# PolarisRisingWar/rgb-experiment

Hardware: AMD Instinct MI355X
Metric: aggregated edges/sec (full-graph GCN d=128, reference epoch = train fwd+bwd+Adam + 2 eval fwd) (higher is better)
Workload: dtype f32

## Files before the change

rgb_experiment_amd/csrc/gemm.hip:

```cpp
#include "rgbx_common.h"

namespace rgbx {
namespace {

constexpr int BM = 128, BN = 128, KT = 32;
enum { A_PLAIN = 0, A_BN = 1, A_ROWS = 2 };

struct TnExtra {
  const float* X;
  int64_t ldx;
  const float *mean, *rstd, *ca, *cb, *ck;
  const int32_t* rows;
  int64_t n_rows;
};
using f32x16 = __attribute__((ext_vector_type(16))) float;

template <int W>
__device__ __forceinline__ void stage_tile(float* __restrict__ lds, const float* __restrict__ src,
                                           int64_t ld, int64_t k0, int64_t k_end, int c0, int ncols) {
  const int tid = threadIdx.x;
#pragma unroll 4
  for (int p = 0; p < KT * W / 256; ++p) {
    const int idx = p * 256 + tid;
    const int r = idx / W, c = idx % W;
    const int64_t k = k0 + r;
    lds[r * W + c] = (k < k_end && c0 + c < ncols) ? src[k * ld + c0 + c] : 0.f;
  }
}

template <int W>
__device__ __forceinline__ void fetch_tile(float4 (&regs)[KT * (W / 4) / 256], const float* __restrict__ src, int64_t ld,
                                           int64_t k0, int64_t k_end, int c0, int ncols) {
#pragma unroll
  for (int p = 0; p < KT * (W / 4) / 256; ++p) {
    const int idx = p * 256 + threadIdx.x;
    const int r = idx / (W / 4), c = (idx % (W / 4)) * 4;
    const int64_t k = k0 + r;
    regs[p] = make_float4(0.f, 0.f, 0.f, 0.f);
    if (k < k_end && c0 + c < ncols) regs[p] = *reinterpret_cast<const float4*>(src + k * ld + c0 + c);
  }
}

template <int W>
__device__ __forceinline__ void put_tile(float* __restrict__ lds, const float4 (&regs)[KT * (W / 4) / 256]) {
#pragma unroll
  for (int p = 0; p < KT * (W / 4) / 256; ++p) {
    const int idx = p * 256 + threadIdx.x;
    const int r = idx / (W / 4), c = (idx % (W / 4)) * 4;
    *reinterpret_cast<float4*>(lds + r * W + c) = regs[p];
  }
}

template <int W>
__device__ __forceinline__ void put_tile_bn(float* __restrict__ lds, const float4 (&rg)[KT * (W / 4) / 256],
                                            const float4 (&rx)[KT * (W / 4) / 256], const float* __restrict__ lc,
                                            int64_t k0, int64_t k_end, int c0, int ncols) {
#pragma unroll
  for (int p = 0; p < KT * (W / 4) / 256; ++p) {
    const int idx = p * 256 + threadIdx.x;
    const int r = idx / (W / 4), c = (idx % (W / 4)) * 4;
    float4 v = rg[p];
    if (k0 + r < k_end && c0 + c < ncols) {
      const float4 mu = *reinterpret_cast<const float4*>(lc + 0 * W + c);
      const float4 rs = *reinterpret_cast<const float4*>(lc + 1 * W + c);
      const float4 a = *reinterpret_cast<const float4*>(lc + 2 * W + c);
      const float4 b = *reinterpret_cast<const float4*>(lc + 3 * W + c);
      const float4 k = *reinterpret_cast<const float4*>(lc + 4 * W + c);
      v.x = bn_bwd_input_grad(v.x, rx[p].x, mu.x, rs.x, a.x, b.x, k.x);
      v.y = bn_bwd_input_grad(v.y, rx[p].y, mu.y, rs.y, a.y, b.y, k.y);
      v.z = bn_bwd_input_grad(v.z, rx[p].z, mu.z, rs.z, a.z, b.z, k.z);
      v.w = bn_bwd_input_grad(v.w, rx[p].w, mu.w, rs.w, a.w, b.w, k.w);
    }
    *reinterpret_cast<float4*>(lds + r * W + c) = v;
  }
}

template <int W>
__device__ __forceinline__ void fetch_row_ids(int32_t (&ids)[KT * (W / 4) / 256], const int32_t* __restrict__ rows,
                                              int64_t j0, int64_t j_end) {
#pragma unroll
  for (int p = 0; p < KT * (W / 4) / 256; ++p) {
    const int64_t j = j0 + (p * 256 + (int)threadIdx.x) / (W / 4);
    ids[p] = j < j_end ? rows[j] : -1;
  }
}

template <int W>
__device__ __forceinline__ void fetch_tile_rows(float4 (&regs)[KT * (W / 4) / 256], const float* __restrict__ src,
                                                int64_t ld, const int32_t (&ids)[KT * (W / 4) / 256], int c0, int ncols) {
#pragma unroll
  for (int p = 0; p < KT * (W / 4) / 256; ++p) {
    const int c = ((p * 256 + (int)threadIdx.x) % (W / 4)) * 4;
    regs[p] = make_float4(0.f, 0.f, 0.f, 0.f);
    if (ids[p] >= 0 && c0 + c < ncols) regs[p] = *reinterpret_cast<const float4*>(src + (int64_t)ids[p] * ld + c0 + c);
  }
}

__device__ __forceinline__ int64_t lower_bound_rows(const int32_t* __restrict__ rows, int64_t n, int64_t key) {
  int64_t lo = 0, hi = n;
  while (lo < hi) {
    const int64_t mid = (lo + hi) >> 1;
    if (rows[mid] < key) lo = mid + 1; else hi = mid;
  }
  return lo;
}

template <bool VEC4, int MT, int MODE = A_PLAIN>
__global__ void __launch_bounds__(256)
gemm_tn_partial_kernel(const float* __restrict__ A, int64_t lda, const float* __restrict__ B, int64_t ldb,
                       float* __restrict__ part, float* __restrict__ colpart, int64_t K, int M, int N,
                       int64_t slab, TnExtra ex) {
  static_assert(MODE == A_PLAIN || VEC4, "the A_BN / A_ROWS forms exist on the 16-byte path only");
  constexpr int MI = MT / 64;
  __shared__ float lds[KT * (MT + 128) + (MODE == A_BN ? 5 * MT : 0)];
  float* la = lds;
  float* lb = lds + KT * MT;
  const int split = blockIdx.x;
  const int m0 = blockIdx.y * MT, n0 = blockIdx.z * BN;
  const int64_t k_begin = (int64_t)split * slab;
  const int64_t k_end = k_begin + slab < K ? k_begin + slab : K;
  const int wave = threadIdx.x >> 6, lane = threadIdx.x & 63;
  const int wm = (wave >> 1) * (MT / 2), wn = (wave & 1) * 64;
  const int kr = lane >> 5, cc = lane & 31;

  f32x16 acc[MI][2];
#pragma unroll
  for (int i = 0; i < MI; ++i)
#pragma unroll
    for (int j = 0; j < 2; ++j)
#pragma unroll
      for (int r = 0; r < 16; ++r) acc[i][j][r] = 0.f;

  const bool sums = colpart != nullptr && blockIdx.z == 0 && threadIdx.x < MT;
  float csum = 0.f;
  auto consume = [&]() {
    if (sums) {
#pragma unroll 8
      for (int r = 0; r < KT; ++r) csum += la[r * MT + threadIdx.x];
    }
#pragma unroll 4
    for (int kk = 0; kk < KT; kk += 2) {
      float a[MI];
#pragma unroll
      for (int i = 0; i < MI; ++i) a[i] = la[(kk + kr) * MT + wm + i * 32 + cc];
      const float b0 = lb[(kk + kr) * 128 + wn + cc];
      const float b1 = lb[(kk + kr) * 128 + wn + 32 + cc];
#pragma unroll
      for (int i = 0; i < MI; ++i) {
        acc[i][0] = __builtin_amdgcn_mfma_f32_32x32x2f32(a[i], b0, acc[i][0], 0, 0, 0);
        acc[i][1] = __builtin_amdgcn_mfma_f32_32x32x2f32(a[i], b1, acc[i][1], 0, 0, 0);
      }
    }
  };
  if constexpr (MODE == A_BN) {
    float* lc = lds + KT * (MT + 128);
    for (int i = threadIdx.x; i < 5 * MT; i += 256) {
      const float* src = i < MT ? ex.mean : i < 2 * MT ? ex.rstd : i < 3 * MT ? ex.ca : i < 4 * MT ? ex.cb : ex.ck;
      const int c = m0 + i % MT;
      lc[i] = c < M ? src[c] : 0.f;
    }
    float4 ra[KT * (MT / 4) / 256], rx[KT * (MT / 4) / 256], rb[KT * 32 / 256];
    fetch_tile<MT>(ra, A, lda, k_begin, k_end, m0, M);
    fetch_tile<MT>(rx, ex.X, ex.ldx, k_begin, k_end, m0, M);
    fetch_tile<128>(rb, B, ldb, k_begin, k_end, n0, N);
    for (int64_t k0 = k_begin; k0 < k_end; k0 += KT) {
      __syncthreads();
      put_tile_bn<MT>(la, ra, rx, lc, k0, k_end, m0, M);
      put_tile<128>(lb, rb);
      __syncthreads();
      if (k0 + KT < k_end) {
        fetch_tile<MT>(ra, A, lda, k0 + KT, k_end, m0, M);
        fetch_tile<MT>(rx, ex.X, ex.ldx, k0 + KT, k_end, m0, M);
        fetch_tile<128>(rb, B, ldb, k0 + KT, k_end, n0, N);
      }
      consume();
    }
  } else if constexpr (MODE == A_ROWS) {
    const int64_t j_begin = lower_bound_rows(ex.rows, ex.n_rows, k_begin);
    const int64_t j_end = lower_bound_rows(ex.rows, ex.n_rows, k_end);
    float4 ra[KT * (MT / 4) / 256], rb[KT * 32 / 256];
    int32_t ia[KT * (MT / 4) / 256], ib[KT * 32 / 256];
    fetch_row_ids<MT>(ia, ex.rows, j_begin, j_end);
    fetch_row_ids<128>(ib, ex.rows, j_begin, j_end);
    fetch_tile_rows<MT>(ra, A, lda, ia, m0, M);
    fetch_tile_rows<128>(rb, B, ldb, ib, n0, N);
    fetch_row_ids<MT>(ia, ex.rows, j_begin + KT, j_end);
    fetch_row_ids<128>(ib, ex.rows, j_begin + KT, j_end);
    for (int64_t j0 = j_begin; j0 < j_end; j0 += KT) {
      __syncthreads();
      put_tile<MT>(la, ra);
      put_tile<128>(lb, rb);
      __syncthreads();
      if (j0 + KT < j_end) {
        fetch_tile_rows<MT>(ra, A, lda, ia, m0, M);
        fetch_tile_rows<128>(rb, B, ldb, ib, n0, N);
        fetch_row_ids<MT>(ia, ex.rows, j0 + 2 * KT, j_end);
        fetch_row_ids<128>(ib, ex.rows, j0 + 2 * KT, j_end);
      }
      consume();
    }
  } else if constexpr (VEC4) {
    float4 ra[KT * (MT / 4) / 256], rb[KT * 32 / 256];
    fetch_tile<MT>(ra, A, lda, k_begin, k_end, m0, M);
    fetch_tile<128>(rb, B, ldb, k_begin, k_end, n0, N);
    for (int64_t k0 = k_begin; k0 < k_end; k0 += KT) {
      __syncthreads();
      put_tile<MT>(la, ra);
      put_tile<128>(lb, rb);
      __syncthreads();
      if (k0 + KT < k_end) {
        fetch_tile<MT>(ra, A, lda, k0 + KT, k_end, m0, M);
        fetch_tile<128>(rb, B, ldb, k0 + KT, k_end, n0, N);
      }
      consume();
    }
  } else {
    for (int64_t k0 = k_begin; k0 < k_end; k0 += KT) {
      __syncthreads();
      stage_tile<MT>(la, A, lda, k0, k_end, m0, M);
      stage_tile<128>(lb, B, ldb, k0, k_end, n0, N);
      __syncthreads();
      consume();
    }
  }

  if (sums && m0 + (int)threadIdx.x < M) colpart[(int64_t)split * M + m0 + threadIdx.x] = csum;
  float* out = part + (int64_t)split * M * N;
#pragma unroll
  for (int i = 0; i < MI; ++i)
#pragma unroll
    for (int j = 0; j < 2; ++j)
#pragma unroll
      for (int r = 0; r < 16; ++r) {
        const int m = m0 + wm + i * 32 + (r & 3) + 8 * (r >> 2) + 4 * kr;
        const int n = n0 + wn + j * 32 + cc;
        if (m < M && n < N) out[(int64_t)m * N + n] = acc[i][j][r];
      }
}

__global__ void __launch_bounds__(256)
gemm_tn_reduce_kernel(const float* __restrict__ part, int S, int64_t MN, float* __restrict__ C, int N,
                      int64_t ldc, float alpha) {
  __shared__ float sh[8][32];
  const int j = threadIdx.x & 31, q = threadIdx.x >> 5;
  for (int64_t base = (int64_t)blockIdx.x * 32; base < MN; base += (int64_t)gridDim.x * 32) {
    const int64_t i = base + j;
    float s = 0.f;
    if (i < MN)
      for (int p = q; p < S; p += 8) s += part[(int64_t)p * MN + i];
    __syncthreads();
    sh[q][j] = s;
    __syncthreads();
    if (q == 0 && i < MN) {
      float t = 0.f;
#pragma unroll
      for (int k = 0; k < 8; ++k) t += sh[k][j];
      C[(i / N) * ldc + (i % N)] = alpha * t;
    }
  }
}

int tile_rows(int M) { return M <= 64 ? 64 : BM; }

int choose_splits(int64_t K, int M, int N) {
  const int64_t tiles = cdiv(M, tile_rows(M)) * cdiv(N, BN);
  int64_t s = cdiv(tile_rows(M) == 64 ? 1024 : 768, tiles);
  const int64_t max_s = cdiv(K, 16 * KT);
  if (s > max_s) s = max_s;
  if (s < 1) s = 1;
  return (int)s;
}

}
}

using namespace rgbx;

extern "C" int rgbx_gemm_tn_workspace_bytes(int64_t K, int64_t M, int64_t N, size_t* bytes) {
  if (!bytes || K < 0 || M < 0 || N < 0) return fail(RGBX_E_ARG, "gemm_tn_workspace_bytes: bad argument");
  if (M >= INT32_MAX || N >= INT32_MAX) return fail(RGBX_E_RANGE, "gemm_tn: M or N exceeds int32");
  *bytes = (size_t)choose_splits(K, (int)M, (int)N) * ((size_t)M * (size_t)N + (size_t)M) * sizeof(float);
  return RGBX_OK;
}

namespace rgbx {
namespace {

int run_gemm_tn(const char* name, int mode, const float* A, int64_t lda, const float* B, int64_t ldb, float* C,
                int64_t ldc, float* a_colsum, int64_t K, int64_t M, int64_t N, float alpha, void* workspace,
                size_t workspace_bytes, rgbx_stream_t stream, const TnExtra& ex) {
  if (K < 0 || M < 0 || N < 0) return fail(RGBX_E_ARG, "%s: negative size", name);
  if (M == 0 || N == 0) return RGBX_OK;
  if (!C || (K > 0 && (!A || !B))) return fail(RGBX_E_ARG, "%s: null pointer", name);
  if (M >= INT32_MAX || N >= INT32_MAX) return fail(RGBX_E_RANGE, "%s: M or N exceeds int32", name);
  if (lda < M || ldb < N || ldc < N) return fail(RGBX_E_ARG, "%s: leading dimension too small", name);
  bool v4 = aligned16(A) && aligned16(B) && lda % 4 == 0 && ldb % 4 == 0;
  if (mode == A_BN) {
    if (K > 0 && (!ex.X || !ex.mean || !ex.rstd || !ex.ca || !ex.cb || !ex.ck))
      return fail(RGBX_E_ARG, "%s: null pointer", name);
    if (ex.ldx < M) return fail(RGBX_E_ARG, "%s: leading dimension too small", name);
    v4 = v4 && aligned16(ex.X) && ex.ldx % 4 == 0;
  }
  if (mode == A_ROWS) {
    if (ex.n_rows < 0 || ex.n_rows > K || (ex.n_rows > 0 && !ex.rows)) return fail(RGBX_E_ARG, "%s: bad row list", name);
    if (K >= INT32_MAX) return fail(RGBX_E_RANGE, "%s: K exceeds int32", name);
  }
  if (mode != A_PLAIN && !v4)
    return fail(RGBX_E_ALIGN, "%s: operands must be 16-byte aligned with leading dimensions that are multiples of 4", name);
  size_t need = 0;
  if (int rc = rgbx_gemm_tn_workspace_bytes(K, M, N, &need)) return rc;
  if (!workspace || workspace_bytes < need)
    return fail(RGBX_E_WS, "%s: workspace %zu < %zu bytes", name, workspace_bytes, need);
  hipStream_t s = (hipStream_t)stream;
  const int S = choose_splits(K, (int)M, (int)N);
  const int64_t slab = cdiv(cdiv(K > 0 ? K : 1, S), KT) * KT;
  float* part = static_cast<float*>(workspace);
  float* colpart = a_colsum ? part + (size_t)S * M * N : nullptr;
  const int mt = tile_rows((int)M);
  dim3 grid(S, (unsigned)cdiv(M, mt), (unsigned)cdiv(N, BN));
#define RGBX_GEMM_TN(V4, MT, MODE) \
  gemm_tn_partial_kernel<V4, MT, MODE><<<grid, 256, 0, s>>>(A, lda, B, ldb, part, colpart, K, (int)M, (int)N, slab, ex)
  if (mode == A_BN) { if (mt == 64) RGBX_GEMM_TN(true, 64, A_BN); else RGBX_GEMM_TN(true, 128, A_BN); }
  else if (mode == A_ROWS) { if (mt == 64) RGBX_GEMM_TN(true, 64, A_ROWS); else RGBX_GEMM_TN(true, 128, A_ROWS); }
  else if (v4) { if (mt == 64) RGBX_GEMM_TN(true, 64, A_PLAIN); else RGBX_GEMM_TN(true, 128, A_PLAIN); }
  else { if (mt == 64) RGBX_GEMM_TN(false, 64, A_PLAIN); else RGBX_GEMM_TN(false, 128, A_PLAIN); }
#undef RGBX_GEMM_TN
  RGBX_CHECK_LAUNCH("gemm_tn_partial_kernel");
  const int64_t MN = M * N;
  int64_t rb = cdiv(MN, 32);
  if (rb > kMaxGrid) rb = kMaxGrid;
  gemm_tn_reduce_kernel<<<(int)rb, 256, 0, s>>>(part, S, MN, C, (int)N, ldc, alpha);
  RGBX_CHECK_LAUNCH("gemm_tn_reduce_kernel");
  if (a_colsum) {
    gemm_tn_reduce_kernel<<<(int)cdiv(M, 32), 256, 0, s>>>(colpart, S, M, a_colsum, (int)M, M, 1.0f);
    RGBX_CHECK_LAUNCH("gemm_tn_reduce_kernel");
  }
  return RGBX_OK;
}

}
}

extern "C" int rgbx_gemm_tn_f32(const float* A, int64_t lda, const float* B, int64_t ldb, float* C,
                                int64_t ldc, float* a_colsum, int64_t K, int64_t M, int64_t N, float alpha,
                                void* workspace, size_t workspace_bytes, rgbx_stream_t stream) {
  return run_gemm_tn("gemm_tn", A_PLAIN, A, lda, B, ldb, C, ldc, a_colsum, K, M, N, alpha, workspace, workspace_bytes,
                     stream, TnExtra{});
}

extern "C" int rgbx_gemm_tn_bn_bwd_f32(const float* G, int64_t ldg, const float* X, int64_t ldx, const float* mean,
                                       const float* rstd, const float* ca, const float* cb, const float* ck,
                                       const float* B, int64_t ldb, float* C, int64_t ldc, float* a_colsum, int64_t K,
                                       int64_t M, int64_t N, float alpha, void* workspace, size_t workspace_bytes,
                                       rgbx_stream_t stream) {
  TnExtra ex{};
  ex.X = X, ex.ldx = ldx, ex.mean = mean, ex.rstd = rstd, ex.ca = ca, ex.cb = cb, ex.ck = ck;
  return run_gemm_tn("gemm_tn_bn_bwd", A_BN, G, ldg, B, ldb, C, ldc, a_colsum, K, M, N, alpha, workspace,
                     workspace_bytes, stream, ex);
}

extern "C" int rgbx_gemm_tn_rows_f32(const float* A, int64_t lda, const float* B, int64_t ldb, const int32_t* rows,
                                     int64_t n_rows, float* C, int64_t ldc, float* a_colsum, int64_t K, int64_t M,
                                     int64_t N, float alpha, void* workspace, size_t workspace_bytes,
                                     rgbx_stream_t stream) {
  TnExtra ex{};
  ex.rows = rows, ex.n_rows = n_rows;
  return run_gemm_tn("gemm_tn_rows", A_ROWS, A, lda, B, ldb, C, ldc, a_colsum, K, M, N, alpha, workspace,
                     workspace_bytes, stream, ex);
}
```

Before: 17.06 billion.

## Software-pipeline MFMA LDS reads, set waves_per_eu, and merge split-K reductions

Adds a rotated consume loop for the 128-row tile that prefetches the next k-step's A/B operands from LDS between MFMA issues, pinned in place with sched_barrier, so LDS latency overlaps matrix work. Sets an amdgpu_waves_per_eu hint (3 for the BN 128-tile variant, 1 otherwise) to steer register allocation. The split-K reduce kernel now handles both the C reduction and the column-sum reduction in a single launch, and unrolls its partial-sum loads 8-way to raise memory-level parallelism. The gains depend on the compiler honouring the scheduling barriers, and the waves_per_eu hint may change occupancy.

```diff
diff --git a/rgb_experiment_amd/csrc/gemm.hip b/rgb_experiment_amd/csrc/gemm.hip
--- a/rgb_experiment_amd/csrc/gemm.hip
+++ b/rgb_experiment_amd/csrc/gemm.hip
@@ -106,7 +106,7 @@
 }
 
 template <bool VEC4, int MT, int MODE = A_PLAIN>
-__global__ void __launch_bounds__(256)
+__global__ void __launch_bounds__(256) __attribute__((amdgpu_waves_per_eu(MODE == A_BN && MT == 128 ? 3 : 1)))
 gemm_tn_partial_kernel(const float* __restrict__ A, int64_t lda, const float* __restrict__ B, int64_t ldb,
                        float* __restrict__ part, float* __restrict__ colpart, int64_t K, int M, int N,
                        int64_t slab, TnExtra ex) {
@@ -152,6 +152,36 @@
       }
     }
   };
+  auto consume_rotate = [&]() {
+    constexpr int I1 = MI - 1;
+    if (sums) {
+#pragma unroll 8
+      for (int r = 0; r < KT; ++r) csum += la[r * MT + threadIdx.x];
+    }
+    const float* pa = la + kr * MT + wm + cc;
+    const float* pb = lb + kr * 128 + wn + cc;
+    float a0 = pa[0], a1 = pa[I1 * 32], b0 = pb[0], b1 = pb[32];
+#pragma unroll
+    for (int kk = 2; kk <= KT; kk += 2) {
+      const bool more = kk < KT;
+      __builtin_amdgcn_sched_barrier(0);
+      acc[0][0] = __builtin_amdgcn_mfma_f32_32x32x2f32(a0, b0, acc[0][0], 0, 0, 0);
+      acc[0][1] = __builtin_amdgcn_mfma_f32_32x32x2f32(a0, b1, acc[0][1], 0, 0, 0);
+      __builtin_amdgcn_sched_barrier(0);
+      if (more) a0 = pa[kk * MT];
+      __builtin_amdgcn_sched_barrier(0);
+      acc[I1][0] = __builtin_amdgcn_mfma_f32_32x32x2f32(a1, b0, acc[I1][0], 0, 0, 0);
+      __builtin_amdgcn_sched_barrier(0);
+      if (more) b0 = pb[kk * 128];
+      __builtin_amdgcn_sched_barrier(0);
+      acc[I1][1] = __builtin_amdgcn_mfma_f32_32x32x2f32(a1, b1, acc[I1][1], 0, 0, 0);
+      __builtin_amdgcn_sched_barrier(0);
+      if (more) {
+        b1 = pb[kk * 128 + 32];
+        a1 = pa[kk * MT + I1 * 32];
+      }
+    }
+  };
   if constexpr (MODE == A_BN) {
     float* lc = lds + KT * (MT + 128);
     for (int i = threadIdx.x; i < 5 * MT; i += 256) {
@@ -173,7 +203,7 @@
         fetch_tile<MT>(rx, ex.X, ex.ldx, k0 + KT, k_end, m0, M);
         fetch_tile<128>(rb, B, ldb, k0 + KT, k_end, n0, N);
       }
-      consume();
+      if constexpr (MI == 2) consume_rotate(); else consume();
     }
   } else if constexpr (MODE == A_ROWS) {
     const int64_t j_begin = lower_bound_rows(ex.rows, ex.n_rows, k_begin);
@@ -197,7 +227,7 @@
         fetch_row_ids<MT>(ia, ex.rows, j0 + 2 * KT, j_end);
         fetch_row_ids<128>(ib, ex.rows, j0 + 2 * KT, j_end);
       }
-      consume();
+      if constexpr (MI == 2) consume_rotate(); else consume();
     }
   } else if constexpr (VEC4) {
     float4 ra[KT * (MT / 4) / 256], rb[KT * 32 / 256];
@@ -212,7 +242,7 @@
         fetch_tile<MT>(ra, A, lda, k0 + KT, k_end, m0, M);
         fetch_tile<128>(rb, B, ldb, k0 + KT, k_end, n0, N);
       }
-      consume();
+      if constexpr (MI == 2) consume_rotate(); else consume();
     }
   } else {
     for (int64_t k0 = k_begin; k0 < k_end; k0 += KT) {
@@ -238,16 +268,39 @@
       }
 }
 
+struct TnReduce {
+  const float* part;
+  int64_t MN;
+  float* out;
+  int N;
+  int64_t ld;
+  float alpha;
+};
+
 __global__ void __launch_bounds__(256)
-gemm_tn_reduce_kernel(const float* __restrict__ part, int S, int64_t MN, float* __restrict__ C, int N,
-                      int64_t ldc, float alpha) {
+gemm_tn_reduce_kernel(TnReduce c, TnReduce sums, int S, int c_blocks) {
   __shared__ float sh[8][32];
+  const bool second = (int)blockIdx.x >= c_blocks;
+  const TnReduce& job = second ? sums : c;
+  const int64_t first = second ? (int)blockIdx.x - c_blocks : (int)blockIdx.x;
+  const int64_t step = second ? (int)gridDim.x - c_blocks : c_blocks;
+  const float* __restrict__ part = job.part;
+  const int64_t MN = job.MN;
   const int j = threadIdx.x & 31, q = threadIdx.x >> 5;
-  for (int64_t base = (int64_t)blockIdx.x * 32; base < MN; base += (int64_t)gridDim.x * 32) {
+  for (int64_t base = first * 32; base < MN; base += step * 32) {
     const int64_t i = base + j;
     float s = 0.f;
-    if (i < MN)
-      for (int p = q; p < S; p += 8) s += part[(int64_t)p * MN + i];
+    if (i < MN) {
+      int p = q;
+      for (; p + 56 < S; p += 64) {
+        float v[8];
+#pragma unroll
+        for (int u = 0; u < 8; ++u) v[u] = part[(int64_t)(p + 8 * u) * MN + i];
+#pragma unroll
+        for (int u = 0; u < 8; ++u) s += v[u];
+      }
+      for (; p < S; p += 8) s += part[(int64_t)p * MN + i];
+    }
     __syncthreads();
     sh[q][j] = s;
     __syncthreads();
@@ -255,7 +308,7 @@
       float t = 0.f;
 #pragma unroll
       for (int k = 0; k < 8; ++k) t += sh[k][j];
-      C[(i / N) * ldc + (i % N)] = alpha * t;
+      job.out[(i / job.N) * job.ld + (i % job.N)] = job.alpha * t;
     }
   }
 }
@@ -329,12 +382,11 @@
   const int64_t MN = M * N;
   int64_t rb = cdiv(MN, 32);
   if (rb > kMaxGrid) rb = kMaxGrid;
-  gemm_tn_reduce_kernel<<<(int)rb, 256, 0, s>>>(part, S, MN, C, (int)N, ldc, alpha);
+  const TnReduce red_c{part, MN, C, (int)N, ldc, alpha};
+  const TnReduce red_sums{colpart, a_colsum ? M : 0, a_colsum, (int)M, M, 1.0f};
+  const int64_t sb = a_colsum ? cdiv(M, 32) : 0;
+  gemm_tn_reduce_kernel<<<(int)(rb + sb), 256, 0, s>>>(red_c, red_sums, S, (int)rb);
   RGBX_CHECK_LAUNCH("gemm_tn_reduce_kernel");
-  if (a_colsum) {
-    gemm_tn_reduce_kernel<<<(int)cdiv(M, 32), 256, 0, s>>>(colpart, S, M, a_colsum, (int)M, M, 1.0f);
-    RGBX_CHECK_LAUNCH("gemm_tn_reduce_kernel");
-  }
   return RGBX_OK;
 }
 
```

Result: no change. 17.16 billion (median of 6 runs) (+0.6%).
